# WU-CVGL/VicaSplat

Hardware: AMD Instinct MI355X
Metric: scenes/sec (8-view 256x256) encode+rasterize (higher is better)
Workload: dtype f32 (f32 activations; products as 3 x f16 MFMA on hi+lo operand pairs, f32 accumulate); 1 GPU; re10k_8view full pipeline fwd: ViT-L encoder+decoder+DPT heads -> 524288 Gaussians/scene, 12 target views/scene rasterized at 256x256; scenes_per_gpu=24, context_views=8, target_views=12, parallelism=scene-sharded x1 (no collective)

## Files before the change

### vicasplat_amd/csrc/stem_stream.hip

```cpp
#include "common.h"
#include "gemm_common.h"

namespace {

struct StemStreamArgs {
    const float *img;
    const float *w;
    const float *bias;
    const float *trunk;
    float *out;
    int N, H, W, Hp, Wp;
    float w_scale, inv_scale;
};

constexpr int kIP = 96;
constexpr int kIS = 16 * kIP;
constexpr int kImgBytes = 2 * 4 * 3 * kIS;

__global__ void __launch_bounds__(512) stem_up_stream_kernel(const StemStreamArgs a) {
    constexpr int PT = 2;
    __shared__ __attribute__((aligned(16))) unsigned char sImg[kImgBytes];
    const int tid = threadIdx.x, lane = tid & 63;
    const int wid = __builtin_amdgcn_readfirstlane(tid >> 6);
    const int l16 = lane & 15, g = lane >> 4;
    const int chb = wid * 32;

    uint4 wh[2][6], wl[2][6];
#pragma unroll
    for (int ct = 0; ct < 2; ++ct)
#pragma unroll
        for (int ks = 0; ks < 6; ++ks) {
            const int q = ks * 4 + g, c = q / 7, kx = q - c * 7;
            const float *wp = a.w + (long long)(chb + ct * 16 + l16) * 147 + c * 49 + kx;
            float v[8];
#pragma unroll
            for (int ky = 0; ky < 8; ++ky) v[ky] = (q < 21 && ky < 7) ? wp[ky * 7] * a.w_scale : 0.f;
            uint4 f0 = make_uint4(__float_as_uint(v[0]), __float_as_uint(v[1]), __float_as_uint(v[2]), __float_as_uint(v[3]));
            uint4 f1 = make_uint4(__float_as_uint(v[4]), __float_as_uint(v[5]), __float_as_uint(v[6]), __float_as_uint(v[7]));
            split8(f0, f1);
            wh[ct][ks] = f0; wl[ct][ks] = f1;
        }
    float bv[2][4];
#pragma unroll
    for (int ct = 0; ct < 2; ++ct) {
        const float4 t = *reinterpret_cast<const float4 *>(a.bias + chb + ct * 16 + 4 * g);
        bv[ct][0] = t.x; bv[ct][1] = t.y; bv[ct][2] = t.z; bv[ct][3] = t.w;
    }
    int ioff[6];
#pragma unroll
    for (int ks = 0; ks < 6; ++ks) {
        int q = ks * 4 + g;
        if (q >= 21) q = 0;
        const int c = q / 7, kx = q - c * 7;
        ioff[ks] = ((kx & 3) * 3 + c) * kIS + ((kx & ~3) + (l16 & 3) * 4) * 2;
    }
    const int trq = l16 >> 2;
    typedef short tr4 __attribute__((ext_vector_type(4)));
    typedef tr4 __attribute__((address_space(3))) *trp_t;
    auto trd = [&](const unsigned char *p) -> uint2 {
        return __builtin_bit_cast(uint2, __builtin_amdgcn_ds_read_tr16_b64_v4i16((trp_t)(const_cast<unsigned char *>(p))));
    };

    const int spx = tid / 3, sc = tid - spx * 3;
    const bool stager = tid < 132;
    auto store_px = [&](int slot, float v) {
        const unsigned h = cvt_pk_f16(v, 0.f) & 0xffffu;
        const _Float16 hf = __builtin_bit_cast(_Float16, (unsigned short)h);
        const unsigned l = cvt_pk_f16(v - (float)hf, 0.f) & 0xffffu;
#pragma unroll
        for (int s = 0; s < 4; ++s) {
            const int j = spx - s;
            if (j >= 0 && j < 48) {
                *reinterpret_cast<unsigned short *>(sImg + (s * 3 + sc) * kIS + slot * kIP + j * 2) = (unsigned short)h;
                *reinterpret_cast<unsigned short *>(sImg + kImgBytes / 2 + (s * 3 + sc) * kIS + slot * kIP + j * 2) = (unsigned short)l;
            }
        }
    };
    for (int i = tid; i < kImgBytes / 4; i += 512) reinterpret_cast<unsigned *>(sImg)[i] = 0u;

    const int Hs = a.H >> 1, Ws = a.W >> 1, C = 256;
    const float ry = (float)(Hs - 1) / (float)(a.H - 1), rx = (float)(Ws - 1) / (float)(a.W - 1);
    const int strips = a.W / (16 * PT), nitems = a.N * strips;
    for (int item = blockIdx.x; item < nitems; item += gridDim.x) {
        const int n = item / strips, x0s = (item - n * strips) * (16 * PT);
        const float *ib = a.img + ((long long)n * a.Hp * a.Wp + x0s) * 3 + tid;
        const bool colok = stager && x0s + spx < a.Wp;
        auto load_row = [&](int r) -> float { return (colok && r < a.Hp) ? ib[(long long)r * a.Wp * 3] : 0.f; };
        __syncthreads();
        float nx[4];
        if (stager) {
#pragma unroll 1
            for (int r0_ = 0; r0_ < 12; r0_ += 4) {
#pragma unroll
                for (int r = 0; r < 4; ++r) nx[r] = load_row(r0_ + r);
#pragma unroll
                for (int r = 0; r < 4; ++r) store_px(r0_ + r, nx[r]);
            }
#pragma unroll
            for (int r = 0; r < 4; ++r) nx[r] = load_row(12 + r);
        }
        int tx0[PT], tx1[PT];
        float tlx[PT];
#pragma unroll
        for (int pt = 0; pt < PT; ++pt) {
            const float sx = (float)(x0s + pt * 16 + l16) * rx;
            tx0[pt] = min((int)sx, Ws - 1);
            tlx[pt] = sx - (float)tx0[pt];
            tx1[pt] = min(tx0[pt] + 1, Ws - 1);
        }
        float4 tpA[2][4], tpB[2][4];
        auto load_taps = [&](float4 (&t)[2][4], const float *q0, const float *q1, int pt) {
#pragma unroll
            for (int ct = 0; ct < 2; ++ct) {
                t[ct][0] = *reinterpret_cast<const float4 *>(q0 + (long long)tx0[pt] * C + ct * 16);
                t[ct][1] = *reinterpret_cast<const float4 *>(q0 + (long long)tx1[pt] * C + ct * 16);
                t[ct][2] = *reinterpret_cast<const float4 *>(q1 + (long long)tx0[pt] * C + ct * 16);
                t[ct][3] = *reinterpret_cast<const float4 *>(q1 + (long long)tx1[pt] * C + ct * 16);
            }
        };
        const float *r0 = a.trunk + ((long long)(n * Hs) * Ws) * C + chb + 4 * g;
        const float *r1 = a.trunk + ((long long)(n * Hs + min(1, Hs - 1)) * Ws) * C + chb + 4 * g;
        float ly_c = 0.f;
        bool same_prev = false;
        load_taps(tpA, r0, r1, 0);
        for (int yo = 0; yo < a.H; ++yo) {
            if ((yo & 3) == 0) {
                if (yo > 0 && stager) {
#pragma unroll
                    for (int r = 0; r < 4; ++r) store_px((yo + 8 + r) & 15, nx[r]);
                }
                __syncthreads();
                if (stager) {
#pragma unroll
                    for (int r = 0; r < 4; ++r) nx[r] = load_row(yo + 12 + r);
                }
            }
            const float ly = ly_c;
            const int so0 = ((yo + trq) & 15) * kIP, so1 = ((yo + 4 + trq) & 15) * kIP;
            const float sy_n = (float)(yo + 1) * ry;
            const int y0_n = min((int)sy_n, Hs - 1), y1_n = min(y0_n + 1, Hs - 1);
            const float *r0_n = a.trunk + ((long long)(n * Hs + y0_n) * Ws) * C + chb + 4 * g, *r1_n = a.trunk + ((long long)(n * Hs + y1_n) * Ws) * C + chb + 4 * g;
            const bool same_next = r0_n == r0 && r1_n == r1;
#pragma unroll
            for (int pt = 0; pt < PT; ++pt) {
                float4 (&tc)[2][4] = (pt & 1) ? tpB : tpA;
                float4 (&tn)[2][4] = (pt & 1) ? tpA : tpB;
                if (pt + 1 < PT) { if (!same_prev) load_taps(tn, r0, r1, pt + 1); }
                else if (yo + 1 < a.H && !same_next) load_taps(tn, r0_n, r1_n, 0);
                f4 acc[2] = {f4{0.f, 0.f, 0.f, 0.f}, f4{0.f, 0.f, 0.f, 0.f}};
#pragma unroll
                for (int ks = 0; ks < 6; ++ks) {
                    const unsigned char *p = sImg + ioff[ks] + pt * 32;
                    const uint2 h0 = trd(p + so0), h1 = trd(p + so1), l0 = trd(p + kImgBytes / 2 + so0), l1 = trd(p + kImgBytes / 2 + so1);
                    const uint4 bh = make_uint4(h0.x, h0.y, h1.x, h1.y), bl = make_uint4(l0.x, l0.y, l1.x, l1.y);
#pragma unroll
                    for (int ct = 0; ct < 2; ++ct) {
                        acc[ct] = mfma<0>(wl[ct][ks], bh, acc[ct]);
                        acc[ct] = mfma<0>(wh[ct][ks], bl, acc[ct]);
                        acc[ct] = mfma<0>(wh[ct][ks], bh, acc[ct]);
                    }
                }
                const float lx = tlx[pt];
                float v[2][4];
#pragma unroll
                for (int ct = 0; ct < 2; ++ct) {
                    const float4 t00 = tc[ct][0], t01 = tc[ct][1], t10 = tc[ct][2], t11 = tc[ct][3];
                    const float a00[4] = {t00.x, t00.y, t00.z, t00.w}, a01[4] = {t01.x, t01.y, t01.z, t01.w};
                    const float a10[4] = {t10.x, t10.y, t10.z, t10.w}, a11[4] = {t11.x, t11.y, t11.z, t11.w};
#pragma unroll
                    for (int r = 0; r < 4; ++r) {
                        const float top = a00[r] * (1.f - lx) + a01[r] * lx, bot = a10[r] * (1.f - lx) + a11[r] * lx;
                        const float st = fmaxf(acc[ct][r] * a.inv_scale + bv[ct][r], 0.f);
                        v[ct][r] = top * (1.f - ly) + bot * ly + st;
                    }
                }
                float *rowp = a.out + ((long long)(n * a.H + yo) * a.W + x0s + pt * 16 + l16) * C;
                store_split8(rowp, chb + 4 * g, v[0], v[1]);
            }
            r0 = r0_n; r1 = r1_n; same_prev = same_next;
            ly_c = sy_n - (float)y0_n;
        }
    }
}

}

extern "C" int vs_stem7x7_up_split_stream(const float *img_padded, const float *w, int32_t w_scale_exp, const float *bias, const float *trunk, void *out,
                                          int32_t N, int32_t H, int32_t W, int32_t Hp, int32_t Wp, int32_t Cout, int32_t nwg, vs_stream_t stream) {
    VS_CHECK(img_padded && w && bias && trunk && out, "vs_stem7x7_up_split_stream: null pointer");
    VS_CHECK(N > 0 && H > 0 && W > 0 && H % 2 == 0 && W % 32 == 0, "vs_stem7x7_up_split_stream: H=%d must be even and W=%d a multiple of 32", H, W);
    VS_CHECK(Cout == 256, "vs_stem7x7_up_split_stream: Cout=%d must be 256", Cout);
    VS_CHECK(Hp >= H + 6 && Wp >= W + 6, "vs_stem7x7_up_split_stream: padded image must be at least (H+6) x (W+6), got %d x %d", Hp, Wp);
    VS_CHECK(nwg >= 1 && nwg <= 65535 && w_scale_exp >= -60 && w_scale_exp <= 60, "vs_stem7x7_up_split_stream: nwg / w_scale_exp out of range");
    VS_CHECK((((uintptr_t)out | (uintptr_t)trunk | (uintptr_t)bias) & 15) == 0, "vs_stem7x7_up_split_stream: out, trunk and bias must be 16-byte aligned");
    VS_CHECK((long long)N * H * W < 2147483647LL, "vs_stem7x7_up_split_stream: too large");
    StemStreamArgs a;
    a.img = img_padded; a.w = w; a.bias = bias; a.trunk = trunk; a.out = (float *)out;
    a.N = N; a.H = H; a.W = W; a.Hp = Hp; a.Wp = Wp;
    a.w_scale = ldexpf(1.f, w_scale_exp); a.inv_scale = ldexpf(1.f, -w_scale_exp);
    hipLaunchKernelGGL(stem_up_stream_kernel, dim3((unsigned)nwg), dim3(512), 0, (hipStream_t)stream, a);
    VS_HIP(hipGetLastError());
    return 0;
}
```

### vicasplat_amd/csrc/conv.hip

```cpp
#include <type_traits>

#include "gemm256.h"
#include "routes.h"

__device__ __attribute__((aligned(128))) unsigned short vs_zero_page[64] = {0};

namespace {

struct ConvArgs {
    const unsigned short *in;
    const unsigned short *w;
    const float *bias;
    const unsigned short *res;
    unsigned short *out;
    int Nimg, H, W, Cin, Cout;
    int relu_in, relu_out;
    int Hin, Win, stride;
    const unsigned short *w2;
    const float *bias2;
    unsigned short *out2;
    int C2, C2pad, ld2;
    float acc_scale;
    float acc_scale2;
    int a_packed;
// ... 240 lines not shown
                const uint4 xf = *reinterpret_cast<const uint4 *>(sX + row * 256 + (((ks * 4 + grp) ^ (row & 15)) << 4));
#pragma unroll
                for (int n = 0; n < NF; ++n) acc2[a_][n] = mfma<BF16>(wf[n], xf, acc2[a_][n]);
            }
        }
    }
    const bool odd = grp & 1;
    const size_t m = (size_t)m0 + wid * 32 + (odd ? 16 : 0) + mrow;
    unsigned short *dst = g.out2 + m * g.ld2 + (grp & ~1) * 4;
    const bool wide = g.ld2 % 8 == 0 && (reinterpret_cast<uintptr_t>(g.out2) & 15) == 0;
#pragma unroll
    for (int n = 0; n < NF; ++n) {
        const float4 b2 = *reinterpret_cast<const float4 *>(g.bias2 + n * 16 + grp * 4);
        uint2 pk[2];
#pragma unroll
        for (int a_ = 0; a_ < 2; ++a_) {
            pk[a_].x = pack16x2<BF16>(acc2[a_][n][0] + b2.x, acc2[a_][n][1] + b2.y);
            pk[a_].y = pack16x2<BF16>(acc2[a_][n][2] + b2.z, acc2[a_][n][3] + b2.w);
        }
        if (wide) {
            const u2v_ sx = __builtin_amdgcn_permlane16_swap(pk[0].x, pk[1].x, false, false);
            const u2v_ sy = __builtin_amdgcn_permlane16_swap(pk[0].y, pk[1].y, false, false);
            *reinterpret_cast<uint4 *>(dst + n * 16) = make_uint4(sx.x, sy.x, sx.y, sy.y);
        } else {
#pragma unroll
            for (int a_ = 0; a_ < 2; ++a_)
                *reinterpret_cast<uint2 *>(g.out2 + ((size_t)m0 + wid * 32 + a_ * 16 + mrow) * g.ld2 + grp * 4 + n * 16) = pk[a_];
        }
    }
}

template <int NF>
__device__ __forceinline__ void conv_head1x1_split_epilogue256(const ConvArgs &g, f4 (&acc)[8][4], int m0, int wr, int wc, unsigned char *smem, int wid,
                                                               int lane) {
    const int mrow = lane & 15, grp = lane >> 4, tid = wid * 64 + lane;
    unsigned char *sXh = smem, *sXl = smem + 32 * 1024, *sW = smem + 64 * 1024;
    f4 acc2[2][NF];
#pragma unroll
    for (int a_ = 0; a_ < 2; ++a_)
#pragma unroll
        for (int n = 0; n < NF; ++n) acc2[a_][n] = f4{0.f, 0.f, 0.f, 0.f};
    const bool relu = g.relu_out == 1;
#pragma unroll
    for (int q = 0; q < 4; ++q) {
        if (q > 0) __syncthreads();
        {
            constexpr int kPieces = NF * 16 * 16;
#pragma unroll
            for (int r = 0; r < (kPieces + 511) / 512; ++r) {
                const int p = r * 512 + tid;
                if (p < kPieces) {
                    const int row = p >> 4, ch = p & 15;
                    const uint4 v = *reinterpret_cast<const uint4 *>(reinterpret_cast<const unsigned char *>(g.w2) + (size_t)row * (g.Cout * 4) + q * 256 + ch * 16);
                    *reinterpret_cast<uint4 *>(sW + row * 256 + ((ch ^ (row & 15)) << 4)) = v;
                }
            }
        }
        if (wc == q) {
            float4 bv[4];
#pragma unroll
            for (int j = 0; j < 4; ++j)
                bv[j] = g.bias ? *reinterpret_cast<const float4 *>(g.bias + wc * 64 + j * 16 + grp * 4) : make_float4(0.f, 0.f, 0.f, 0.f);
#pragma unroll
            for (int i = 0; i < 8; ++i) {
                const int row = wr * 128 + i * 16 + mrow;
#pragma unroll
                for (int j = 0; j < 4; ++j) {
                    float v0 = acc[i][j][0] * g.acc_scale + bv[j].x, v1 = acc[i][j][1] * g.acc_scale + bv[j].y;
                    float v2 = acc[i][j][2] * g.acc_scale + bv[j].z, v3 = acc[i][j][3] * g.acc_scale + bv[j].w;
                    if (relu) { v0 = fmaxf(v0, 0.f); v1 = fmaxf(v1, 0.f); v2 = fmaxf(v2, 0.f); v3 = fmaxf(v3, 0.f); }
                    const unsigned h0 = cvt_pk_f16(v0, v1), h1 = cvt_pk_f16(v2, v3);
                    float r0, r1, r2, r3;
                    asm("v_fma_mix_f32 %0, %1, -1.0, %2 op_sel_hi:[1,0,0]" : "=v"(r0) : "v"(h0), "v"(v0));
                    asm("v_fma_mix_f32 %0, %1, -1.0, %2 op_sel:[1,0,0] op_sel_hi:[1,0,0]" : "=v"(r1) : "v"(h0), "v"(v1));
                    asm("v_fma_mix_f32 %0, %1, -1.0, %2 op_sel_hi:[1,0,0]" : "=v"(r2) : "v"(h1), "v"(v2));
                    asm("v_fma_mix_f32 %0, %1, -1.0, %2 op_sel:[1,0,0] op_sel_hi:[1,0,0]" : "=v"(r3) : "v"(h1), "v"(v3));
                    const unsigned l0 = cvt_pk_f16(r0, r1), l1 = cvt_pk_f16(r2, r3);
                    const int chunk = ((j >> 1) * 4 + grp) ^ ((row >> 1) & 7);
                    const int off = row * 128 + chunk * 16 + (j & 1) * 8;
                    *reinterpret_cast<uint2 *>(sXh + off) = make_uint2(h0, h1);
                    *reinterpret_cast<uint2 *>(sXl + off) = make_uint2(l0, l1);
                }
            }
        }
        __syncthreads();
#pragma unroll
        for (int ks = 0; ks < 2; ++ks) {
            uint4 xh[2], xl[2];
#pragma unroll
            for (int a_ = 0; a_ < 2; ++a_) {
                const int row = wid * 32 + a_ * 16 + mrow;
                const int o = row * 128 + (((ks * 4 + grp) ^ ((row >> 1) & 7)) << 4);
                xh[a_] = *reinterpret_cast<const uint4 *>(sXh + o); xl[a_] = *reinterpret_cast<const uint4 *>(sXl + o);
            }
#pragma unroll
            for (int n = 0; n < NF; ++n) {
                const int row = n * 16 + mrow;
                const uint4 wh = *reinterpret_cast<const uint4 *>(sW + row * 256 + (((ks * 8 + grp) ^ (row & 15)) << 4));
                const uint4 wl = *reinterpret_cast<const uint4 *>(sW + row * 256 + (((ks * 8 + 4 + grp) ^ (row & 15)) << 4));
#pragma unroll
                for (int a_ = 0; a_ < 2; ++a_) acc2[a_][n] = mma2<kDtSplit>(wh, wl, xh[a_], xl[a_], acc2[a_][n]);
            }
        }
    }
    float *out2 = reinterpret_cast<float *>(g.out2);
#pragma unroll
    for (int n = 0; n < NF; ++n) {
        const float4 b2 = *reinterpret_cast<const float4 *>(g.bias2 + n * 16 + grp * 4);
#pragma unroll
        for (int a_ = 0; a_ < 2; ++a_) {
            const size_t m = (size_t)m0 + wid * 32 + a_ * 16 + mrow;
            *reinterpret_cast<float4 *>(out2 + m * g.ld2 + n * 16 + grp * 4) =
                make_float4(acc2[a_][n][0] * g.acc_scale2 + b2.x, acc2[a_][n][1] * g.acc_scale2 + b2.y, acc2[a_][n][2] * g.acc_scale2 + b2.z,
                            acc2[a_][n][3] * g.acc_scale2 + b2.w);
        }
    }
}

struct ConvStager256 {
    const unsigned short *pa[2][2];
    const unsigned short *pz[2];
    unsigned vmask[2][2];
    const unsigned short *pw[2][2];
    int Cin, Win, kpt;
    __device__ __forceinline__ void stage(int u, int kt, unsigned lds) const {
        if (u < 2) {
            const int kc = (kt * 7282) >> 16, tap = kt - kc * 9;
            const int ty = (tap * 11) >> 5;
            const int dy = ty - 1, dx = tap - ty * 3 - 1;
            const long long off = (long long)(dy * Win + dx) * Cin + kc * 64;
#pragma unroll
            for (int j = 0; j < 2; ++j) {
                const bool ok = (vmask[u][j] >> tap) & 1u;
                glds16(ok ? pa[u][j] + off : pz[j], lds + j * 1024u);
            }
        } else {
            const int kc = (kt * 7282) >> 16, wk = (kt - kc * 9) * kpt + kc;
            glds16(pw[u - 2][0] + wk * 64, lds);
            glds16(pw[u - 2][1] + wk * 64, lds + 1024u);
        }
    }
};

template <int BF16, bool RELU_IN, int FUSE_NF = 0, bool APACK = false>
// ... 75 lines not shown
    const int wr = wid >> 2, wc = wid & 3;
    const int K = 9 * g.Cin;
    const int tiles_x = g.W >> 4, tiles_img = (g.H >> 4) * tiles_x;
    const int nwg = g.Nimg * tiles_img;
    const int bid = vs::route::xcd_remap(blockIdx.x, nwg);
    const int nimg = bid / tiles_img, trem = bid - nimg * tiles_img;
    const int y0 = (trem / tiles_x) * 16, x0 = (trem % tiles_x) * 16;

    ConvHaloStager st;
    st.K = K; st.kpt = kpt;
    st.img = g.in + (size_t)nimg * g.H * g.W * g.Cin;
    st.wgt = g.w;
    st.zo = (lane & 7) * 8;
    st.pmask = 0;
#pragma unroll
    for (int r = 0; r < 3; ++r)
#pragma unroll
        for (int k = 0; k < 2; ++k) {
            const int p = (r * 8 + wid) * 16 + k * 8 + (lane >> 3);
            const int chunk = (lane & 7) ^ ((p >> 1) & 7);
            const int ry = p / 18, rx = p - ry * 18;
            const int y = y0 - 1 + ry, x = x0 - 1 + rx;
            const bool ok = p < 324 && (unsigned)y < (unsigned)g.H && (unsigned)x < (unsigned)g.W;
            st.po[r][k] = ok ? (unsigned)((y * g.W + x) * g.Cin + chunk * 8) : 0u;
            if (ok) st.pmask |= 1u << (2 * r + k);
        }
    {
        const int q = unit_row256(wid, 0, lane);
        st.wo = (unsigned)(unit_b_tile_row256(q, 0) * K + unit_src_chunk256(q, lane) * 8);
    }
    f4 acc[8][4];
    mainloop256_halo_split<RELU_IN>(st, kpt, acc, smem, lane, wid);
    conv_epilogue<kDtSplit, 8>(g, acc, (nimg * g.H + y0 + wr * 8) * g.W + x0, wc * 64, g.Nimg * g.H * g.W, smem, wid, lane, g.W);
}

struct ConvStager256x128 {
    const unsigned short *pa[2][2];
    const unsigned short *pz[2];
    unsigned vmask[2][2];
    const unsigned short *pw[2];
    int Cin, Win, kpt;
    __device__ __forceinline__ void stage(int u, int kt, unsigned lds) const {
        if (u < 2) {
            const int kc = (kt * 7282) >> 16, tap = kt - kc * 9;
            const int ty = (tap * 11) >> 5;
            const int dy = ty - 1, dx = tap - ty * 3 - 1;
            const long long off = (long long)(dy * Win + dx) * Cin + kc * 64;
#pragma unroll
            for (int j = 0; j < 2; ++j) {
                const bool ok = (vmask[u][j] >> tap) & 1u;
                glds16(ok ? pa[u][j] + off : pz[j], lds + j * 1024u);
            }
        } else {
            const int kc = (kt * 7282) >> 16, wk = (kt - kc * 9) * kpt + kc;
            glds16(pw[0] + wk * 64, lds);
            glds16(pw[1] + wk * 64, lds + 1024u);
        }
    }
};

template <int BF16, int MI>
__device__ __forceinline__ void conv_head_dot_epilogue(const ConvArgs &g, f4 (&acc)[MI][4], int m0, int wr, int wc, float *red, int lane);

template <bool RELU_IN, bool FUSE_DOT, bool A_PACKED = false>
__global__ void __launch_bounds__(512, 1) conv3x3_256x128_split_kernel(const ConvArgs g, const int kpt) {
    __shared__ __attribute__((aligned(1024))) unsigned char smem[2 * 3 * kUnitBytes256];
// ... 602 lines not shown
    ConvArgs g{(const unsigned short *)in, (const unsigned short *)wp, bias, nullptr, nullptr, Nimg, H, W, 2 * Cin, 128, relu_in, relu_out, H, W, 1,
               (const unsigned short *)w2, bias2, (unsigned short *)out2, C2, C2, ld2, acc_scale, 1.f};
    const int cshift = vs::route::conv_cshift(2 * Cin);
    const bool tile128 = cshift >= 0 && (9 * 2 * Cin / 64) % 2 == 0 && !relu_in;
    VS_CHECK(!in_packed || tile128, "vs_conv3x3_head_dot_split_nhwc: a packed input needs the 256 x 128 tile kernel (Cin in {32, 64, 128, 256}, no relu_in)");
    if (tile128 && in_packed)
        hipLaunchKernelGGL((conv3x3_256x128_split_kernel<false, true, true>), dim3((unsigned)(M / 256)), dim3(512), 0, stream, g, 1 << cshift);
    else if (tile128)
        hipLaunchKernelGGL((conv3x3_256x128_split_kernel<false, true>), dim3((unsigned)(M / 256)), dim3(512), 0, stream, g, 1 << cshift);
    else
        hipLaunchKernelGGL((conv3x3_kernel<kDtSplit, 8, true>), dim3((unsigned)(M / 256)), dim3(256), 0, stream, g);
    VS_HIP(hipGetLastError());
    return 0;
}

extern "C" int vs_conv3x3_head1x1_split_nhwc(const float *in, const void *wp, float acc_scale, const float *bias, const void *w2p, float acc_scale2,
                                             const float *bias2, float *out2, int32_t Nimg, int32_t H, int32_t W, int32_t Cin, int32_t C2, int32_t C2pad,
                                             int32_t ld2, int32_t relu_out, vs_stream_t stream_) {
    hipStream_t stream = (hipStream_t)stream_;
    const int in_packed = vs::route::take_packed_flag(relu_out);
    VS_CHECK(in && wp && w2p && bias2 && out2 && acc_scale > 0.f && acc_scale2 > 0.f, "vs_conv3x3_head1x1_split_nhwc: null pointer / bad scale");
    const long long M = (long long)Nimg * H * W;
    VS_CHECK(Nimg > 0 && H > 0 && W > 0 && H < 32767 && W < 65536 && M % 256 == 0 && M < 2147483647LL, "vs_conv3x3_head1x1_split_nhwc: N*H*W must be a positive multiple of 256");
    const int cshift = vs::route::conv_cshift(2 * Cin);
    VS_CHECK(cshift >= 0 && (9 * 2 * Cin / 64) % 2 == 0, "vs_conv3x3_head1x1_split_nhwc: Cin=%d not supported", Cin);
    VS_CHECK(C2pad % 16 == 0 && C2pad >= 16 && C2pad <= 96 && C2 <= C2pad && ld2 >= C2pad && ld2 % 4 == 0 && (relu_out == 0 || relu_out == 1),
             "vs_conv3x3_head1x1_split_nhwc: need C2pad in 16..96 (multiple of 16), ld2 >= C2pad (C2pad=%d ld2=%d)", C2pad, ld2);
    VS_CHECK((((uintptr_t)in | (uintptr_t)wp | (uintptr_t)w2p | (uintptr_t)out2 | (uintptr_t)bias2) & 15) == 0 && (!bias || ((uintptr_t)bias & 15) == 0),
             "vs_conv3x3_head1x1_split_nhwc: 16-byte alignment required");
    ConvArgs g{(const unsigned short *)in, (const unsigned short *)wp, bias, nullptr, nullptr, Nimg, H, W, 2 * Cin, 256, 0, relu_out, H, W, 1,
               (const unsigned short *)w2p, bias2, (unsigned short *)out2, C2, C2pad, ld2, acc_scale, acc_scale2};
    dim3 grid((unsigned)(M / 256)), block(512);
    g.a_packed = in_packed;
    with_head_nf(C2pad, [&](auto nf) {
        if (in_packed) hipLaunchKernelGGL((conv3x3_256_kernel<kDtSplit, false, decltype(nf)::value, true>), grid, block, 0, stream, g, 1 << cshift);
        else hipLaunchKernelGGL((conv3x3_256_kernel<kDtSplit, false, decltype(nf)::value>), grid, block, 0, stream, g, 1 << cshift);
    });
    VS_HIP(hipGetLastError());
    return 0;
}

extern "C" int vs_upsample2x_nhwc(const void *in, const void *add, void *out, int32_t Nimg, int32_t H, int32_t W, int32_t C,
                                  int32_t relu_add, int32_t dtype, vs_stream_t stream_) {
    hipStream_t stream = (hipStream_t)stream_;
    VS_CHECK(in && out, "vs_upsample2x_nhwc: null pointer");
    VS_CHECK(dtype == 1 || dtype == 2 || dtype == 3, "vs_upsample2x_nhwc: dtype must be 1 (f16), 2 (bf16) or 3 (f32)");
    const int pack_out = (relu_add & 16) ? 1 : 0;
    relu_add &= ~16;
    VS_CHECK(!pack_out || (dtype == 3 && C % 32 == 0 && ((uintptr_t)out & 127) == 0), "vs_upsample2x_nhwc: a packed output needs dtype 3, C %% 32 == 0, 128-byte alignment");
    if (dtype == 3) {
        VS_CHECK(C % 4 == 0, "vs_upsample2x_nhwc: C=%d must be a multiple of 4", C);
        if ((long long)Nimg * H * W * C <= 0) return 0;
        if (H >= 2 && W >= 2) {
            const int rows = Nimg * H, gy = rows < 32768 ? rows : 32768;
            hipLaunchKernelGGL(upsample2x_f32_block_kernel, dim3((unsigned)vs::cdiv(W * (C / 4), 256), gy, vs::cdiv(rows, gy)), dim3(256), 0, stream,
                               (const float *)in, (const float *)add, (float *)out, Nimg, H, W, C, relu_add, pack_out);
            VS_HIP(hipGetLastError());
            return 0;
        }
        VS_CHECK(!pack_out, "vs_upsample2x_nhwc: the packed output needs H, W >= 2");
        const int rows = Nimg * 2 * H, gy = rows < 32768 ? rows : 32768;
        hipLaunchKernelGGL(upsample2x_f32_kernel, dim3((unsigned)vs::cdiv(2 * W * (C / 4), 256), gy, vs::cdiv(rows, gy)), dim3(256), 0, stream,
                           (const float *)in, (const float *)add, (float *)out, Nimg, H, W, C, relu_add);
        VS_HIP(hipGetLastError());
        return 0;
    }
    VS_CHECK(C % 8 == 0, "vs_upsample2x_nhwc: C=%d must be a multiple of 8", C);
    if ((long long)Nimg * H * W * C <= 0) return 0;
// ... 23 lines not shown
```

### vicasplat_amd/csrc/gemm256.h

```cpp
#pragma once
#include "gemm_common.h"
#include "routes.h"

namespace {

constexpr unsigned kUnitBytes256 = 128 * 128;
constexpr unsigned kLdsBytes256 = 2 * 4 * kUnitBytes256;

__device__ __forceinline__ int unit_row256(int wid, int j, int lane) { return wid * 16 + j * 8 + (lane >> 3); }
__device__ __forceinline__ int unit_src_chunk256(int q, int lane) { return (lane & 7) ^ ((q >> 1) & 7); }
__device__ __forceinline__ int unit_a_tile_row256(int q, int h) { return (q >> 6) * 128 + h * 64 + (q & 63); }
__device__ __forceinline__ int unit_b_tile_row256(int q, int h) { return (q >> 5) * 64 + h * 32 + (q & 31); }

template <int BF16, bool RELU_A, class Stager, bool TN = false>
__device__ __forceinline__ void mainloop256(Stager &st, const int KT, f4 (&acc)[8][4], const unsigned char *smem, const int lane,
                                            const int wid) {
    static_assert(BF16 != kDtSplit, "split operands run mainloop256_split");
    constexpr unsigned UNITB = kUnitBytes256;
    const int wr = wid >> 2, wc = wid & 3;
    typedef void __attribute__((address_space(3))) *lptr_t;
    const unsigned lds0 = (unsigned)(size_t)(lptr_t)smem;
    const unsigned lds_w = __builtin_amdgcn_readfirstlane(lds0 + (unsigned)wid * 2048u);
#define VS_STAGE(u_, kt_, d_) st.stage(u_, kt_, lds_w + (unsigned)(((d_) * 4 + (u_)) * UNITB));

// ... 237 lines not shown
    VS_BAR()
    VS_CVT_LD(0, 0)
    VS_CVT_ST(0, 0)
    VS_LGK0
    VS_BAR()
    if (wr == 1) VS_BAR()
    for (int kt = 0; kt + 2 < KT; kt += 2) {
        VS_KTILE(kt, 0, 0)
        VS_KTILE(kt + 1, 1, 0)
    }
    VS_KTILE(KT - 2, 0, 1)
    VS_KTILE(KT - 1, 1, 2)
    if (wr == 0) VS_BAR()
#undef VS_KTILE
#undef VS_WAIT
#undef VS_COMPUTE
#undef VS_BAR
#undef VS_MM
#undef VS_CVT_LD
#undef VS_CVT_ST
#undef VS_LGK0
#undef VS_RD_B
#undef VS_RD_A
#undef VS_STAGE
    __syncthreads();
}

constexpr unsigned kHaloPatchBytes = 336 * 128;
constexpr unsigned kHaloDumpOff = 2 * kHaloPatchBytes;
constexpr unsigned kHaloRingOff = kHaloDumpOff + 2048;
constexpr unsigned kLdsBytesHalo = kHaloRingOff + 4 * kUnitBytes256;
static_assert(kHaloRingOff % 1024 == 0, "units are 1 KiB-aligned");

template <bool RELU_A, class Stager>
__device__ __forceinline__ void mainloop256_halo_split(Stager &st, const int NCB, f4 (&acc)[8][4], unsigned char *smem, const int lane, const int wid) {
    constexpr unsigned UNITB = kUnitBytes256;
    constexpr int BF16 = kDtSplit;
    const int wr = wid >> 2, wc = wid & 3;
    typedef void __attribute__((address_space(3))) *lptr_t;
    const unsigned lds0 = (unsigned)(size_t)(lptr_t)smem;
    const unsigned lds_u = __builtin_amdgcn_readfirstlane(lds0);
    const unsigned lds_w = __builtin_amdgcn_readfirstlane(lds0 + (unsigned)wid * 2048u);
    const int frow = lane & 15, fg = lane >> 4;
    const unsigned rd0 = (unsigned)(frow * 128 + (((0 + fg) ^ (frow >> 1)) << 4));
    const unsigned rd1 = (unsigned)(frow * 128 + (((4 + fg) ^ (frow >> 1)) << 4));
    const unsigned char *rdB = smem + kHaloRingOff + wc * (32 * 128);
    unsigned q0 = (unsigned)(wr * 8 * 18 + frow);
    const int crow = 2 * (frow & 7) + (frow >> 3);
    const unsigned cv0 = (unsigned)(crow * 128 + (((0 + fg) ^ (crow >> 1)) << 4));
    const unsigned cv1 = cv0 ^ 64u;
    uint4 fa[4][2], fb[2][2][2], cx0, cx1;
#pragma unroll
    for (int i = 0; i < 8; ++i)
#pragma unroll
        for (int j = 0; j < 4; ++j) acc[i][j] = f4{0.f, 0.f, 0.f, 0.f};

#define VS_STAGE_P(r_, cb_, pb_) st.stage_p(r_, cb_, ((r_) * 8 + wid < 21) ? lds_u + (pb_) + (unsigned)(((r_) * 8 + wid) * 2048) : lds_u + kHaloDumpOff);
#define VS_CVT_P(r_, pb_)                                                                                        \
    if ((r_) * 8 + wid < 21) {                                                                                   \
        unsigned char *cp_ = smem + (pb_) + ((r_) * 8 + wid) * 2048;                                             \
        cx0 = *reinterpret_cast<const uint4 *>(cp_ + cv0);                                                       \
        cx1 = *reinterpret_cast<const uint4 *>(cp_ + cv1);                                                       \
        if constexpr (RELU_A) {                                                                                  \
            cx0.x = relu_f32_lds(cx0.x); cx0.y = relu_f32_lds(cx0.y); cx0.z = relu_f32_lds(cx0.z); cx0.w = relu_f32_lds(cx0.w); \
            cx1.x = relu_f32_lds(cx1.x); cx1.y = relu_f32_lds(cx1.y); cx1.z = relu_f32_lds(cx1.z); cx1.w = relu_f32_lds(cx1.w); \
        }                                                                                                        \
        split8_lds(cx0, cx1);                                                                                    \
        *reinterpret_cast<uint4 *>(cp_ + cv0) = cx0;                                                             \
        *reinterpret_cast<uint4 *>(cp_ + cv1) = cx1;                                                             \
    }
#define VS_STAGE_B(h_, t_, cb_, d_) st.stage_b(h_, t_, cb_, lds_w + kHaloRingOff + (unsigned)(((d_) * 2 + (h_)) * UNITB));
#define VS_RD_A(h_, t_, pb_)                                                                                     \
    _Pragma("unroll") for (int i = 0; i < 4; ++i) {                                                              \
        const unsigned p_ = q0 + (unsigned)(((h_) * 4 + i + (t_) / 3) * 18 + (t_) % 3);                          \
        const unsigned a_ = (pb_) + p_ * 128u + ((((p_ >> 1) ^ (unsigned)fg) & 7u) << 4);                        \
        fa[i][0] = *reinterpret_cast<const uint4 *>(smem + a_);                                                  \
        fa[i][1] = *reinterpret_cast<const uint4 *>(smem + (a_ ^ 64u));                                          \
    }
#define VS_RD_B(h_, d_)                                                                                          \
    _Pragma("unroll") for (int j = 0; j < 2; ++j) {                                                              \
        fb[h_][j][0] = *reinterpret_cast<const uint4 *>(rdB + ((d_) * 2 + (h_)) * UNITB + j * 2048 + rd0);       \
        fb[h_][j][1] = *reinterpret_cast<const uint4 *>(rdB + ((d_) * 2 + (h_)) * UNITB + j * 2048 + rd1);       \
    }
#define VS_LGK0 asm volatile("s_waitcnt lgkmcnt(0)" ::: "memory");
#define VS_MM(ha_, hb_)                                                                                          \
    _Pragma("unroll") for (int i = 0; i < 4; ++i)                                                                \
        _Pragma("unroll") for (int j = 0; j < 2; ++j)                                                            \
            acc[(ha_) * 4 + i][(hb_) * 2 + j] = mma2<BF16>(fb[hb_][j][0], fb[hb_][j][1], fa[i][0], fa[i][1], acc[(ha_) * 4 + i][(hb_) * 2 + j]);
#define VS_BAR()                                  \
    {                                             \
        asm volatile("" ::: "memory");            \
        __builtin_amdgcn_sched_barrier(0);        \
        __builtin_amdgcn_s_barrier();             \
        __builtin_amdgcn_sched_barrier(0);        \
        asm volatile("" ::: "memory");            \
    }
#define VS_WAIT(n_) asm volatile("s_waitcnt vmcnt(" #n_ ")" ::: "memory");
#define VS_COMPUTE(ha_, hb_, g0_wait_, all_wait_) \
    {                                             \
        VS_BAR()                                  \
        __builtin_amdgcn_s_setprio(1);            \
        VS_MM(ha_, hb_)                           \
        __builtin_amdgcn_s_setprio(0);            \
        if (wr == 0) { g0_wait_ }                 \
        all_wait_                                 \
        VS_BAR()                                  \
    }
#define VS_TAPWAIT(MORE_, PST_) { if (MORE_) { if (PST_) { VS_WAIT(6) } else { VS_WAIT(4) } } else { VS_WAIT(0) } }
#define VS_TAP(t_, LAST_)                                                         \
    {                                                                             \
        const int d_ = (cb + (t_)) & 1;                                           \
        constexpr bool more_ = !(LAST_) || (t_) + 2 < 9;                          \
        constexpr bool pst_ = !(LAST_) && (t_) < 3;                               \
        constexpr int t2_ = (t_) + 2 < 9 ? (t_) + 2 : (t_) - 7;                   \
        const int cb2_ = (t_) + 2 < 9 ? cb : cb + 1;                              \
        asm volatile("" : "+v"(q0));    \
        VS_RD_B(0, d_) VS_RD_A(0, t_, pc)                                         \
// ... 583 lines not shown
```

### vicasplat_amd/csrc/routes.h

```cpp
#pragma once
#include <cstdint>

#ifdef __HIPCC__
#define VS_HOST_DEVICE __host__ __device__
#else
#define VS_HOST_DEVICE
#endif

namespace vs {
namespace route {

inline int cdiv(int a, int b) { return (a + b - 1) / b; }
inline long long cdiv64(long long a, long long b) { return (a + b - 1) / b; }

VS_HOST_DEVICE inline int xcd_remap(int bid, int n) {
    const int q = n / 8, r = n % 8, xcd = bid % 8, idx = bid / 8;
    return (xcd < r ? xcd * (q + 1) : r * (q + 1) + (xcd - r) * q) + idx;
}

constexpr int kF32 = 2, kSplit = 3;
enum class Leaf { SmallM, Skinny, G256, Mi2, Mi4, Mi8 };
struct GemmStep { Leaf leaf; int nw, mf, m_lo, m_hi, ksplit; };
struct GemmPlan { int n; GemmStep step[2]; };

// ... 70 lines not shown
        if (Cin2 == (64 << sft)) return sft;
    return -1;
}
inline int take_packed_flag(int32_t &flag) {
    const int packed = (flag & 16) ? 1 : 0;
    flag &= ~16;
    return packed;
}

enum class ConvKind { Halo256, Tile256, Tile256x128, Wave4, PackedNotTaken };
struct ConvRoute { ConvKind kind; int kpt, mi; long long grid; };

inline ConvRoute conv3x3_route(int dtype, long long M, int H, int W, int Cin2, int Cout, int stride, bool a_packed) {
    const int cshift = conv_cshift(Cin2);
    const int kpt_any = (Cin2 % 64 == 0 && Cin2 / 64 <= 64) ? Cin2 / 64 : -1;
    const int kpt = cshift >= 0 ? 1 << cshift : (dtype == 4 && !a_packed ? kpt_any : -1);
    const long long t256 = cdiv64(M, 256) * cdiv(Cout, 256);
    const long long t256_min = dtype == 4 ? 150 : 224;
    if (kpt > 0 && Cout % 256 == 0 && (9 * kpt) % 2 == 0 && t256 >= t256_min) {
        const bool halo = dtype == 4 && stride == 1 && Cout == 256 && H % 16 == 0 && W % 16 == 0 && !a_packed && (long long)H * W * Cin2 < 2147483647LL;
        return {halo ? ConvKind::Halo256 : ConvKind::Tile256, kpt, 0, t256};
    }
    const long long big = cdiv64(M, 256) * cdiv(Cout, 128), t4 = cdiv64(M, 128) * cdiv(Cout, 128);
    if (dtype == 3) return {ConvKind::Wave4, 0, 4, t4};
    if (dtype != 4) return big >= 256 ? ConvRoute{ConvKind::Wave4, 0, 8, big} : ConvRoute{ConvKind::Wave4, 0, 4, t4};
    if (cshift >= 0 && Cout % 128 == 0 && Cout % 256 != 0 && (9 * kpt) % 2 == 0 && big >= 224)
        return {ConvKind::Tile256x128, kpt, 0, cdiv64(M, 256) * (Cout / 128)};
    if (a_packed) return {ConvKind::PackedNotTaken, 0, 0, 0};
    if (big >= 512) return {ConvKind::Wave4, 0, 8, big};
    if (t4 <= 192 && M > 64) return {ConvKind::Wave4, 0, 2, cdiv64(M, 64) * cdiv(Cout, 128)};
    return {ConvKind::Wave4, 0, 4, t4};
}

constexpr int kResMaxKeys = 320, kResMaxQueries = 3 * 8 * 16;
enum class AttnKind { Res, Tile64, Tile128, F32, Split64, Split128, Packed96 };
struct AttnRoute { AttnKind kind; long long gx; int gy, gz, block; };

inline AttnRoute attention_route(int dtype, bool in_packed, int nbatch, int H, int Lq, int Lk, bool has_seg, bool has_len) {
    if (dtype == 4 && in_packed) return {AttnKind::Packed96, (long long)cdiv(Lq, 96) * H * nbatch, 1, 1, 256};
    if (dtype == 3) return {AttnKind::F32, cdiv(Lq, 64), H, nbatch, 256};
    if (dtype != 4 && !has_seg && !has_len && Lk <= kResMaxKeys && Lq <= kResMaxQueries) return {AttnKind::Res, 1, H, nbatch, 512};
    const int Lk_eff = has_seg ? 2 * Lk : Lk;
    const bool big = (long long)cdiv(Lq, 128) * H * nbatch >= 512 && Lk_eff > (dtype == 4 ? 256 : 1024);
    const AttnKind kind = dtype == 4 ? (big ? AttnKind::Split128 : AttnKind::Split64) : (big ? AttnKind::Tile128 : AttnKind::Tile64);
    return {kind, cdiv(Lq, big ? 128 : 64), H, nbatch, 256};
}

struct AttnBwdRoute { int keys, gq, gk; };
inline AttnBwdRoute attention_bwd_route(bool split, int Lq, int Lk, bool has_seg, int max_keys) {
    const int keys = has_seg ? max_keys : Lk;
    return {keys, cdiv(Lq, 128), cdiv(keys, split ? 64 : 128)};
}

}
}
```

Measured before the change: 102.7 scenes/s.

## Stage trunk rows into LDS via async global-to-LDS loads for upsample taps

Replaces per-thread global float4 loads of the bilinear upsample trunk taps with a ring of six trunk rows staged into LDS through async glds16 loads. Rows are prefetched a few output rows ahead, and completion is managed with s_waitcnt vmcnt plus the existing block barrier. This is meant to cut redundant global traffic and hide trunk-read latency behind the MFMA stem convolution. In exchange the kernel uses more LDS per block, which could lower occupancy, and it depends on hand-written vmcnt accounting. Bias registers are pinned with empty asm constraints, and contraction is disabled on the coordinate math so the tap indices and weights match the previous computation.

Result: no change. 103.2 scenes/s, median of 6 (+0.5%).

```diff
diff --git a/vicasplat_amd/csrc/stem_stream.hip b/vicasplat_amd/csrc/stem_stream.hip
--- a/vicasplat_amd/csrc/stem_stream.hip
+++ b/vicasplat_amd/csrc/stem_stream.hip
@@ -16,14 +16,26 @@
 constexpr int kIP = 96;
 constexpr int kIS = 16 * kIP;
 constexpr int kImgBytes = 2 * 4 * 3 * kIS;
+constexpr int kTPix = 18;
+constexpr int kTP = 1024 + 16;
+constexpr int kTRowB = kTPix * kTP;
+constexpr int kTRows = 6;
+constexpr int kTrunkBytes = kTRows * kTRowB;
+#define VS_WAIT(n_) asm volatile("s_waitcnt vmcnt(" #n_ ")" ::: "memory");
 
 __global__ void __launch_bounds__(512) stem_up_stream_kernel(const StemStreamArgs a) {
     constexpr int PT = 2;
-    __shared__ __attribute__((aligned(16))) unsigned char sImg[kImgBytes];
+    __shared__ __attribute__((aligned(16))) unsigned char sMem[kImgBytes + kTrunkBytes];
+    unsigned char *const sImg = sMem;
+    const unsigned char *const sTr = sMem + kImgBytes;
+    typedef void __attribute__((address_space(3))) *lptr_t;
+    const unsigned ldsT = (unsigned)(size_t)(lptr_t)(sMem + kImgBytes);
     const int tid = threadIdx.x, lane = tid & 63;
     const int wid = __builtin_amdgcn_readfirstlane(tid >> 6);
     const int l16 = lane & 15, g = lane >> 4;
     const int chb = wid * 32;
+    const int tsrc_chunk = ((lane >> 4) * 2 + ((lane >> 2) & 1)) * 8 + ((lane >> 1) & 1) * 4 + (lane & 1) * 2 + ((lane >> 3) & 1);
+    const int toff = ((wid >> 1) * 16 + (g & 1) * 8 + (wid & 1) * 4 + (g >> 1)) * 16;
 
     uint4 wh[2][6], wl[2][6];
 #pragma unroll
@@ -46,6 +58,10 @@
         const float4 t = *reinterpret_cast<const float4 *>(a.bias + chb + ct * 16 + 4 * g);
         bv[ct][0] = t.x; bv[ct][1] = t.y; bv[ct][2] = t.z; bv[ct][3] = t.w;
     }
+#pragma unroll
+    for (int ct = 0; ct < 2; ++ct)
+#pragma unroll
+        for (int r = 0; r < 4; ++r) asm volatile("" : "+v"(bv[ct][r]));
     int ioff[6];
 #pragma unroll
     for (int ks = 0; ks < 6; ++ks) {
@@ -87,66 +103,84 @@
         const bool colok = stager && x0s + spx < a.Wp;
         auto load_row = [&](int r) -> float { return (colok && r < a.Hp) ? ib[(long long)r * a.Wp * 3] : 0.f; };
         __syncthreads();
-        float nx[4];
+        const int pb = (x0s >> 1) - 1;
+        const float *tsrc = a.trunk + (long long)n * Hs * Ws * C + tsrc_chunk * 4;
+        auto stage_rows = [&](int lo, int hi) {
+            const int np = (hi - lo + 1) * kTPix;
+            for (int i = wid; i < np; i += 8) {
+                const int r = i / kTPix, p = i - r * kTPix;
+                const int sp = min(max(pb + p, 0), Ws - 1);
+                glds16(tsrc + ((long long)(lo + r) * Ws + sp) * C, __builtin_amdgcn_readfirstlane(ldsT + (unsigned)(((lo + r) % kTRows) * kTRowB + p * kTP)));
+            }
+        };
+        auto need_of = [&](int y) -> int { return __builtin_amdgcn_readfirstlane(min(min((int)((float)y * ry), Hs - 1) + 1, Hs - 1)); };
+        int staged = need_of(min(3, a.H - 1));
+        stage_rows(0, staged);
+        float nx[4] = {0.f, 0.f, 0.f, 0.f};
         if (stager) {
 #pragma unroll 1
             for (int r0_ = 0; r0_ < 12; r0_ += 4) {
-#pragma unroll
-                for (int r = 0; r < 4; ++r) nx[r] = load_row(r0_ + r);
-#pragma unroll
-                for (int r = 0; r < 4; ++r) store_px(r0_ + r, nx[r]);
-            }
-#pragma unroll
-            for (int r = 0; r < 4; ++r) nx[r] = load_row(12 + r);
+                float px[4];
+#pragma unroll
+                for (int r = 0; r < 4; ++r) px[r] = load_row(r0_ + r);
+#pragma unroll
+                for (int r = 0; r < 4; ++r) store_px(r0_ + r, px[r]);
+            }
         }
         int tx0[PT], tx1[PT];
         float tlx[PT];
 #pragma unroll
         for (int pt = 0; pt < PT; ++pt) {
+#pragma clang fp contract(off)
             const float sx = (float)(x0s + pt * 16 + l16) * rx;
             tx0[pt] = min((int)sx, Ws - 1);
             tlx[pt] = sx - (float)tx0[pt];
             tx1[pt] = min(tx0[pt] + 1, Ws - 1);
         }
-        float4 tpA[2][4], tpB[2][4];
-        auto load_taps = [&](float4 (&t)[2][4], const float *q0, const float *q1, int pt) {
+        int to0[PT], to1[PT];
+#pragma unroll
+        for (int pt = 0; pt < PT; ++pt) { to0[pt] = (tx0[pt] - pb) * kTP + toff; to1[pt] = (tx1[pt] - pb) * kTP + toff; }
+        auto read_taps = [&](float4 (&t)[2][4], int s0, int s1, int pt) {
 #pragma unroll
             for (int ct = 0; ct < 2; ++ct) {
-                t[ct][0] = *reinterpret_cast<const float4 *>(q0 + (long long)tx0[pt] * C + ct * 16);
-                t[ct][1] = *reinterpret_cast<const float4 *>(q0 + (long long)tx1[pt] * C + ct * 16);
-                t[ct][2] = *reinterpret_cast<const float4 *>(q1 + (long long)tx0[pt] * C + ct * 16);
-                t[ct][3] = *reinterpret_cast<const float4 *>(q1 + (long long)tx1[pt] * C + ct * 16);
+                t[ct][0] = *reinterpret_cast<const float4 *>(sTr + s0 + to0[pt] + ct * 32);
+                t[ct][1] = *reinterpret_cast<const float4 *>(sTr + s0 + to1[pt] + ct * 32);
+                t[ct][2] = *reinterpret_cast<const float4 *>(sTr + s1 + to0[pt] + ct * 32);
+                t[ct][3] = *reinterpret_cast<const float4 *>(sTr + s1 + to1[pt] + ct * 32);
             }
         };
-        const float *r0 = a.trunk + ((long long)(n * Hs) * Ws) * C + chb + 4 * g;
-        const float *r1 = a.trunk + ((long long)(n * Hs + min(1, Hs - 1)) * Ws) * C + chb + 4 * g;
-        float ly_c = 0.f;
-        bool same_prev = false;
-        load_taps(tpA, r0, r1, 0);
         for (int yo = 0; yo < a.H; ++yo) {
             if ((yo & 3) == 0) {
                 if (yo > 0 && stager) {
 #pragma unroll
                     for (int r = 0; r < 4; ++r) store_px((yo + 8 + r) & 15, nx[r]);
                 }
+                if (yo == 0) VS_WAIT(0) else VS_WAIT(8)
                 __syncthreads();
+                if (yo + 4 < a.H) {
+                    const int nd = need_of(min(yo + 7, a.H - 1));
+                    if (nd > staged) { stage_rows(staged + 1, nd); staged = nd; }
+                }
                 if (stager) {
 #pragma unroll
                     for (int r = 0; r < 4; ++r) nx[r] = load_row(yo + 12 + r);
                 }
             }
-            const float ly = ly_c;
             const int so0 = ((yo + trq) & 15) * kIP, so1 = ((yo + 4 + trq) & 15) * kIP;
-            const float sy_n = (float)(yo + 1) * ry;
-            const int y0_n = min((int)sy_n, Hs - 1), y1_n = min(y0_n + 1, Hs - 1);
-            const float *r0_n = a.trunk + ((long long)(n * Hs + y0_n) * Ws) * C + chb + 4 * g, *r1_n = a.trunk + ((long long)(n * Hs + y1_n) * Ws) * C + chb + 4 * g;
-            const bool same_next = r0_n == r0 && r1_n == r1;
+            int y0;
+            float ly;
+            {
+#pragma clang fp contract(off)
+                const float sy = (float)yo * ry;
+                y0 = min((int)sy, Hs - 1);
+                ly = sy - (float)y0;
+            }
+            const int y1 = min(y0 + 1, Hs - 1);
+            const int ts0 = (y0 % kTRows) * kTRowB, ts1 = (y1 % kTRows) * kTRowB;
 #pragma unroll
             for (int pt = 0; pt < PT; ++pt) {
-                float4 (&tc)[2][4] = (pt & 1) ? tpB : tpA;
-                float4 (&tn)[2][4] = (pt & 1) ? tpA : tpB;
-                if (pt + 1 < PT) { if (!same_prev) load_taps(tn, r0, r1, pt + 1); }
-                else if (yo + 1 < a.H && !same_next) load_taps(tn, r0_n, r1_n, 0);
+                float4 tc[2][4];
+                read_taps(tc, ts0, ts1, pt);
                 f4 acc[2] = {f4{0.f, 0.f, 0.f, 0.f}, f4{0.f, 0.f, 0.f, 0.f}};
 #pragma unroll
                 for (int ks = 0; ks < 6; ++ks) {
@@ -177,8 +211,6 @@
                 float *rowp = a.out + ((long long)(n * a.H + yo) * a.W + x0s + pt * 16 + l16) * C;
                 store_split8(rowp, chb + 4 * g, v[0], v[1]);
             }
-            r0 = r0_n; r1 = r1_n; same_prev = same_next;
-            ly_c = sy_n - (float)y0_n;
         }
     }
 }
```

## Route packed DPT head 3x3 conv through halo-tiled kernel with async W2 staging

Applied to the files above, without the earlier changes.

Adds a halo-tiled 3x3 conv kernel for the fused conv+1x1 head path when the input is pre-packed hi/lo. Each block covers a 16x16 spatial tile and loads an 18x18 halo once instead of re-gathering per tap, and it skips the in-loop split conversion because the operand is already packed. The head epilogue now stages the second-GEMM weights with global_load_lds (direct global-to-LDS) rather than going through registers, and it takes a row stride so the 16x16 tile maps back to image rows. This adds a new kernel and routing condition, and it relies on hand-written waitcnt and m0 asm being correct.

Result: no change. 103.6 scenes/s before, 103.9 scenes/s after (median of 5 runs) (+0.3%).

```diff
diff --git a/vicasplat_amd/csrc/conv.hip b/vicasplat_amd/csrc/conv.hip
--- a/vicasplat_amd/csrc/conv.hip
+++ b/vicasplat_amd/csrc/conv.hip
@@ -296,8 +296,8 @@
 
 template <int NF>
 __device__ __forceinline__ void conv_head1x1_split_epilogue256(const ConvArgs &g, f4 (&acc)[8][4], int m0, int wr, int wc, unsigned char *smem, int wid,
-                                                               int lane) {
-    const int mrow = lane & 15, grp = lane >> 4, tid = wid * 64 + lane;
+                                                               int lane, const int istep = 16) {
+    const int mrow = lane & 15, grp = lane >> 4;
     unsigned char *sXh = smem, *sXl = smem + 32 * 1024, *sW = smem + 64 * 1024;
     f4 acc2[2][NF];
 #pragma unroll
@@ -305,26 +305,32 @@
 #pragma unroll
         for (int n = 0; n < NF; ++n) acc2[a_][n] = f4{0.f, 0.f, 0.f, 0.f};
     const bool relu = g.relu_out == 1;
+    typedef void __attribute__((address_space(3))) *lptr_t;
+    const unsigned lds_sw = __builtin_amdgcn_readfirstlane((unsigned)(size_t)(lptr_t)sW);
+    const unsigned w2_off = (unsigned)((wid * 4 + grp) * (g.Cout * 4) + (((lane & 15) ^ ((wid * 4 + grp) & 15)) << 4));
+    auto stage_w2 = [&](const int q) {
+        constexpr int kInstr = NF * 4;
+#pragma unroll
+        for (int r = 0; r < (kInstr + 7) / 8; ++r) {
+            const int it = r * 8 + wid;
+            if (it < kInstr) {
+                const unsigned char *base = reinterpret_cast<const unsigned char *>(g.w2) + (size_t)(r * 32) * (g.Cout * 4) + q * 256;
+                asm volatile("s_mov_b32 m0, %0\n\ts_nop 0\n\tglobal_load_lds_dwordx4 %1, %2" ::"s"(lds_sw + (unsigned)it * 1024u),
+                             "v"(w2_off), "s"(base) : "memory");
+            }
+        }
+    };
 #pragma unroll
     for (int q = 0; q < 4; ++q) {
         if (q > 0) __syncthreads();
-        {
-            constexpr int kPieces = NF * 16 * 16;
-#pragma unroll
-            for (int r = 0; r < (kPieces + 511) / 512; ++r) {
-                const int p = r * 512 + tid;
-                if (p < kPieces) {
-                    const int row = p >> 4, ch = p & 15;
-                    const uint4 v = *reinterpret_cast<const uint4 *>(reinterpret_cast<const unsigned char *>(g.w2) + (size_t)row * (g.Cout * 4) + q * 256 + ch * 16);
-                    *reinterpret_cast<uint4 *>(sW + row * 256 + ((ch ^ (row & 15)) << 4)) = v;
-                }
-            }
-        }
+        stage_w2(q);
         if (wc == q) {
+            const float *bp = g.bias;
+            asm volatile("" : "+s"(bp));
             float4 bv[4];
 #pragma unroll
             for (int j = 0; j < 4; ++j)
-                bv[j] = g.bias ? *reinterpret_cast<const float4 *>(g.bias + wc * 64 + j * 16 + grp * 4) : make_float4(0.f, 0.f, 0.f, 0.f);
+                bv[j] = bp ? *reinterpret_cast<const float4 *>(bp + wc * 64 + j * 16 + grp * 4) : make_float4(0.f, 0.f, 0.f, 0.f);
 #pragma unroll
             for (int i = 0; i < 8; ++i) {
                 const int row = wr * 128 + i * 16 + mrow;
@@ -347,6 +353,7 @@
                 }
             }
         }
+        asm volatile("s_waitcnt vmcnt(0)" ::: "memory");
         __syncthreads();
 #pragma unroll
         for (int ks = 0; ks < 2; ++ks) {
@@ -373,7 +380,7 @@
         const float4 b2 = *reinterpret_cast<const float4 *>(g.bias2 + n * 16 + grp * 4);
 #pragma unroll
         for (int a_ = 0; a_ < 2; ++a_) {
-            const size_t m = (size_t)m0 + wid * 32 + a_ * 16 + mrow;
+            const size_t m = (size_t)m0 + (size_t)((wid * 2 + a_) * istep + mrow);
             *reinterpret_cast<float4 *>(out2 + m * g.ld2 + n * 16 + grp * 4) =
                 make_float4(acc2[a_][n][0] * g.acc_scale2 + b2.x, acc2[a_][n][1] * g.acc_scale2 + b2.y, acc2[a_][n][2] * g.acc_scale2 + b2.z,
                             acc2[a_][n][3] * g.acc_scale2 + b2.w);
@@ -515,6 +522,62 @@
     f4 acc[8][4];
     mainloop256_halo_split<RELU_IN>(st, kpt, acc, smem, lane, wid);
     conv_epilogue<kDtSplit, 8>(g, acc, (nimg * g.H + y0 + wr * 8) * g.W + x0, wc * 64, g.Nimg * g.H * g.W, smem, wid, lane, g.W);
+}
+
+struct ConvHaloHeadStager : ConvHaloStager {
+    __device__ __forceinline__ void stage_p(int r, int cb, unsigned lds) const {
+#pragma unroll
+        for (int k = 0; k < 2; ++k) {
+            const bool ok = (pmask >> (2 * r + k)) & 1u;
+            unsigned o = po[r][k];
+            asm volatile("" : "+v"(o));
+            glds16(ok ? img + (o + (unsigned)(cb * 64)) : vs_zero_page, lds + k * 1024u);
+        }
+    }
+};
+
+template <int NF>
+__global__ void __launch_bounds__(512, 1) conv3x3_256_halo_head_split_kernel(const ConvArgs g, const int kpt) {
+    __shared__ __attribute__((aligned(1024))) unsigned char smem[kLdsBytesHalo];
+    static_assert(64 * 1024 + NF * 16 * 256 <= kLdsBytesHalo, "the second GEMM's X and W2 images fit the block");
+    const int tid = threadIdx.x, lane = tid & 63;
+    const int wid = __builtin_amdgcn_readfirstlane(tid >> 6);
+    const int wr = wid >> 2, wc = wid & 3;
+    const int K = 9 * g.Cin;
+    const int tiles_x = g.W >> 4, tiles_img = (g.H >> 4) * tiles_x;
+    const int nwg = g.Nimg * tiles_img;
+    const int bid = vs::route::xcd_remap(blockIdx.x, nwg);
+    const int nimg = bid / tiles_img, trem = bid - nimg * tiles_img;
+    const int y0 = (trem / tiles_x) * 16, x0 = (trem % tiles_x) * 16;
+
+    ConvHaloHeadStager st;
+    st.K = K; st.kpt = kpt;
+    st.img = g.in + (size_t)nimg * g.H * g.W * g.Cin;
+    st.wgt = g.w;
+    st.zo = (lane & 7) * 8;
+    st.pmask = 0;
+#pragma unroll
+    for (int r = 0; r < 3; ++r)
+#pragma unroll
+        for (int k = 0; k < 2; ++k) {
+            const int p = (r * 8 + wid) * 16 + k * 8 + (lane >> 3);
+            const int chunk = (lane & 7) ^ ((p >> 1) & 7);
+            const int ry = p / 18, rx = p - ry * 18;
+            const int y = y0 - 1 + ry, x = x0 - 1 + rx;
+            const bool ok = p < 324 && (unsigned)y < (unsigned)g.H && (unsigned)x < (unsigned)g.W;
+            unsigned o = ok ? (unsigned)((y * g.W + x) * g.Cin + chunk * 8) : 0u;
+            asm volatile("v_mov_b32 %0, %1" : "=v"(st.po[r][k]) : "v"(o));
+            if (ok) st.pmask |= 1u << (2 * r + k);
+        }
+    {
+        const int q = unit_row256(wid, 0, lane);
+        st.wo = (unsigned)(unit_b_tile_row256(q, 0) * K + unit_src_chunk256(q, lane) * 8);
+    }
+    f4 acc[8][4];
+    mainloop256_halo_split<false, ConvHaloHeadStager, true>(st, kpt, acc, smem, lane, wid);
+    int elane = lane;
+    asm volatile("" : "+v"(elane));
+    conv_head1x1_split_epilogue256<NF>(g, acc, (nimg * g.H + y0) * g.W + x0, wr, wc, smem, wid, elane, g.W);
 }
 
 struct ConvStager256x128 {
@@ -1183,8 +1246,10 @@
                (const unsigned short *)w2p, bias2, (unsigned short *)out2, C2, C2pad, ld2, acc_scale, acc_scale2};
     dim3 grid((unsigned)(M / 256)), block(512);
     g.a_packed = in_packed;
+    const bool halo = vs::route::head_halo_takes(in_packed, H, W, 2 * Cin);
     with_head_nf(C2pad, [&](auto nf) {
-        if (in_packed) hipLaunchKernelGGL((conv3x3_256_kernel<kDtSplit, false, decltype(nf)::value, true>), grid, block, 0, stream, g, 1 << cshift);
+        if (halo) hipLaunchKernelGGL((conv3x3_256_halo_head_split_kernel<decltype(nf)::value>), grid, block, 0, stream, g, 1 << cshift);
+        else if (in_packed) hipLaunchKernelGGL((conv3x3_256_kernel<kDtSplit, false, decltype(nf)::value, true>), grid, block, 0, stream, g, 1 << cshift);
         else hipLaunchKernelGGL((conv3x3_256_kernel<kDtSplit, false, decltype(nf)::value>), grid, block, 0, stream, g, 1 << cshift);
     });
     VS_HIP(hipGetLastError());
diff --git a/vicasplat_amd/csrc/gemm256.h b/vicasplat_amd/csrc/gemm256.h
--- a/vicasplat_amd/csrc/gemm256.h
+++ b/vicasplat_amd/csrc/gemm256.h
@@ -293,8 +293,9 @@
 constexpr unsigned kLdsBytesHalo = kHaloRingOff + 4 * kUnitBytes256;
 static_assert(kHaloRingOff % 1024 == 0, "units are 1 KiB-aligned");
 
-template <bool RELU_A, class Stager>
+template <bool RELU_A, class Stager, bool A_PACKED = false>
 __device__ __forceinline__ void mainloop256_halo_split(Stager &st, const int NCB, f4 (&acc)[8][4], unsigned char *smem, const int lane, const int wid) {
+    static_assert(!(RELU_A && A_PACKED), "a packed A operand carries its ReLU already");
     constexpr unsigned UNITB = kUnitBytes256;
     constexpr int BF16 = kDtSplit;
     const int wr = wid >> 2, wc = wid & 3;
@@ -308,9 +309,10 @@
     const unsigned char *rdB = smem + kHaloRingOff + wc * (32 * 128);
     unsigned q0 = (unsigned)(wr * 8 * 18 + frow);
     const int crow = 2 * (frow & 7) + (frow >> 3);
-    const unsigned cv0 = (unsigned)(crow * 128 + (((0 + fg) ^ (crow >> 1)) << 4));
-    const unsigned cv1 = cv0 ^ 64u;
-    uint4 fa[4][2], fb[2][2][2], cx0, cx1;
+    [[maybe_unused]] const unsigned cv0 = (unsigned)(crow * 128 + (((0 + fg) ^ (crow >> 1)) << 4));
+    [[maybe_unused]] const unsigned cv1 = cv0 ^ 64u;
+    uint4 fa[4][2], fb[2][2][2];
+    [[maybe_unused]] uint4 cx0, cx1;
 #pragma unroll
     for (int i = 0; i < 8; ++i)
 #pragma unroll
@@ -318,7 +320,7 @@
 
 #define VS_STAGE_P(r_, cb_, pb_) st.stage_p(r_, cb_, ((r_) * 8 + wid < 21) ? lds_u + (pb_) + (unsigned)(((r_) * 8 + wid) * 2048) : lds_u + kHaloDumpOff);
 #define VS_CVT_P(r_, pb_)                                                                                        \
-    if ((r_) * 8 + wid < 21) {                                                                                   \
+    if constexpr (!A_PACKED) if ((r_) * 8 + wid < 21) {                                                          \
         unsigned char *cp_ = smem + (pb_) + ((r_) * 8 + wid) * 2048;                                             \
         cx0 = *reinterpret_cast<const uint4 *>(cp_ + cv0);                                                       \
         cx1 = *reinterpret_cast<const uint4 *>(cp_ + cv1);                                                       \
@@ -343,7 +345,7 @@
         fb[h_][j][0] = *reinterpret_cast<const uint4 *>(rdB + ((d_) * 2 + (h_)) * UNITB + j * 2048 + rd0);       \
         fb[h_][j][1] = *reinterpret_cast<const uint4 *>(rdB + ((d_) * 2 + (h_)) * UNITB + j * 2048 + rd1);       \
     }
-#define VS_LGK0 asm volatile("s_waitcnt lgkmcnt(0)" ::: "memory");
+#define VS_LGK0 if constexpr (!A_PACKED) asm volatile("s_waitcnt lgkmcnt(0)" ::: "memory");
 #define VS_MM(ha_, hb_)                                                                                          \
     _Pragma("unroll") for (int i = 0; i < 4; ++i)                                                                \
         _Pragma("unroll") for (int j = 0; j < 2; ++j)                                                            \
diff --git a/vicasplat_amd/csrc/routes.h b/vicasplat_amd/csrc/routes.h
--- a/vicasplat_amd/csrc/routes.h
+++ b/vicasplat_amd/csrc/routes.h
@@ -126,6 +126,10 @@
     return {ConvKind::Wave4, 0, 4, t4};
 }
 
+inline bool head_halo_takes(bool a_packed, int H, int W, int Cin2) {
+    return a_packed && H % 16 == 0 && W % 16 == 0 && (long long)H * W * Cin2 < 2147483648LL;
+}
+
 constexpr int kResMaxKeys = 320, kResMaxQueries = 3 * 8 * 16;
 enum class AttnKind { Res, Tile64, Tile128, F32, Split64, Split128, Packed96 };
 struct AttnRoute { AttnKind kind; long long gx; int gy, gz, block; };
```
